# QY-H00/attention-interpolation-diffusion

Hardware: AMD Instinct MI355X
Metric: interpolation-frames/sec (50-step) (higher is better)
Workload: dtype bf16

## Files before the change

attention-interpolation-diffusion_amd/csrc/aid_attn.hip:

```cpp
#include <stdio.h>
#include <stdlib.h>

#include <type_traits>

#include "aid_common.hpp"
#include "aid_kernels.hpp"

namespace aid {

constexpr int KT = 64;
constexpr int VLD = KT + 8;

struct AttnKParams {
    AidAttnArgs a;
    int32_t nqb;
    float   c2;
    int32_t q_iters;
    int32_t skip_single;
};

constexpr int RES_KEYS = 96;
constexpr int RES_VLD = RES_KEYS + 8;
constexpr int RES_SLACK = 64;

// ... 915 lines not shown
                    if (dv < D) {
                        f32x4 v;
#pragma unroll
                        for (int e = 0; e < 4; ++e) v[e] = res[j][d][4 * g + e] * osc;
                        if (a.accumulate) {
                            const f32x4 old = up4<T>(*reinterpret_cast<const T4*>(orow + dv));
                            v += old;
                        }
                        *reinterpret_cast<T4*>(orow + dv) = cvt4<T>(v);
                    }
                }
        }
    }
    if (RES) {
#pragma unroll
        for (int j = 0; j < QB; ++j)
#pragma unroll
            for (int ks = 0; ks < NQK; ++ks) qf[j][ks] = qn[j][ks];
    }
    }
}

template <typename T, int D, int MODE, int NW, int QB, bool PIPE, bool RES = false, bool BIAS = false>
static hipError_t launch_variant(const AttnKParams& p, hipStream_t stream) {
    constexpr int DK = (D + 15) / 16 * 16, DV = (D + 31) / 32 * 32;
    constexpr int NREG = MODE == AID_MODE_PLAIN ? 1 : MODE == AID_MODE_INNER ? 2 : 3;
    const size_t smem = RES ? ((size_t)NREG * (RES_KEYS * (DK + 8) + DV * RES_VLD) + RES_SLACK) * sizeof(T)
                            : (size_t)((attn_prefetch(D, NW) || QB > 1) ? 2 : 1) * (KT * (DK + 8) + DV * VLD) * sizeof(T);
    static PerDevice<int> attr_set;
    const hipError_t e =
        set_max_dynamic_lds(attr_set, 0, reinterpret_cast<const void*>(&aid_attn_kernel<T, D, MODE, NW, QB, PIPE, RES, BIAS>), smem);
    if (e != hipSuccess) return e;
    const int grid = p.nqb * p.a.n_frames * p.a.heads;
    hipLaunchKernelGGL((aid_attn_kernel<T, D, MODE, NW, QB, PIPE, RES, BIAS>), dim3(grid), dim3(NW * 64), smem, stream, p);
    return hipGetLastError();
}

static int attn_qb(const AidAttnArgs& a);

static int attn_nw(const AidAttnArgs& a) {
    const int knob = tune(TUNE_ATTN_NW);
    if (a.d > 80) return 4;
    if (attn_qb(a) >= 2) return 4;
    if (knob >= 0) return knob == 8 ? 8 : 4;
    return (a.d == 64 && a.mode == AID_MODE_OUTER && a.l >= 2048) ? 8 : 4;
}

static int attn_qb(const AidAttnArgs& a) {
    const int force = tune(TUNE_ATTN_QB);
    if (a.d != 40 || a.mode != AID_MODE_PLAIN) return 1;
    if (force == 1 || force == 2) return force;
    return (a.d == 40 && a.mode == AID_MODE_PLAIN && a.s >= 2048 && a.l >= 1024) ? 2 : 1;
}

static bool attn_pipe(const AidAttnArgs& a) {
    const int knob = tune(TUNE_ATTN_PIPE);
    const bool built = a.d == 40 || (a.d == 64 && a.mode == AID_MODE_PLAIN);
    if (!built || a.l < 192) return false;
    return knob > 0;
}

constexpr int RES_CHUNKS_MAX = 8;
static bool attn_res(const AidAttnArgs& a) {
    const int knob = tune(TUNE_ATTN_RES);
    if (a.d > 80 || a.l > RES_KEYS) return false;
    if (knob >= 0) return knob != 0;
    return a.d == 40;
}

template <typename T, int D, int MODE>
static hipError_t launch_order(const AttnStep& st, const AttnKParams& p, hipStream_t stream) {
    constexpr bool SMALL = D <= 80, QB2 = D == 40 && MODE == AID_MODE_PLAIN, CAN_PIPE = D == 40 || (D == 64 && MODE == AID_MODE_PLAIN);
    if (st.bias)             return launch_variant<T, D, MODE, 4, 1, false, false, true>(p, stream);
    if (SMALL && st.res)     return launch_variant<T, D, MODE, 4, 1, false, SMALL>(p, stream);
    if (QB2 && st.qb == 2)   return launch_variant<T, D, MODE, 4, QB2 ? 2 : 1, false>(p, stream);
    if (SMALL && st.nw == 8) return launch_variant<T, D, MODE, SMALL ? 8 : 4, 1, false>(p, stream);
    if (CAN_PIPE && st.pipe) return launch_variant<T, D, MODE, 4, 1, CAN_PIPE>(p, stream);
    const bool base = st.nw == 4 && st.qb == 1 && !st.pipe && !st.res;
    return base ? launch_variant<T, D, MODE, 4, 1, false>(p, stream) : hipErrorInvalidValue;
}

template <typename T>
static hipError_t launch_order(const AttnStep& st, const AttnKParams& p, hipStream_t stream) {
    static_assert(AID_MODE_PLAIN == 0 && AID_MODE_INNER == 1 && AID_MODE_OUTER == 2, "mode index");
    typedef hipError_t (*Fn)(const AttnStep&, const AttnKParams&, hipStream_t);
    static const Fn by_d_mode[4][3] = {{launch_order<T, 40, 0>, launch_order<T, 40, 1>, launch_order<T, 40, 2>},
                                       {launch_order<T, 64, 0>, launch_order<T, 64, 1>, launch_order<T, 64, 2>},
                                       {launch_order<T, 80, 0>, launch_order<T, 80, 1>, launch_order<T, 80, 2>},
                                       {launch_order<T, 160, 0>, launch_order<T, 160, 1>, launch_order<T, 160, 2>}};
    const int di = p.a.d == 40 ? 0 : p.a.d == 64 ? 1 : p.a.d == 80 ? 2 : p.a.d == 160 ? 3 : -1;
    return di < 0 ? hipErrorInvalidValue : by_d_mode[di][p.a.mode](st, p, stream);
}

template <typename T>
__global__ __launch_bounds__(256) void aid_lerp_kv_kernel(const T* __restrict__ k, const T* __restrict__ vt,
                                                          T* __restrict__ k2, T* __restrict__ vt2,
                                                          const float* __restrict__ coef, int n_frames, int begin,
                                                          int end, int64_t k_fs, int64_t vt_fs) {
    typedef typename Vec<T>::v8 T8;
    const int fr = blockIdx.y;
    const float c = coef[fr];
    if (c <= 0.f || c >= 1.f) return;
    const int64_t nk8 = k_fs / 8, nv8 = vt_fs / 8;
    for (int64_t i = (int64_t)blockIdx.x * blockDim.x + threadIdx.x; i < nk8 + nv8; i += (int64_t)gridDim.x * blockDim.x) {
        const bool isk = i < nk8;
        const int64_t j = isk ? i : i - nk8;
        const T* src = isk ? k : vt;
        const int64_t fs = isk ? k_fs : vt_fs;
        const f32x8 x0 = up8<T>(*reinterpret_cast<const T8*>(src + begin * fs + j * 8));
        const f32x8 x1 = up8<T>(*reinterpret_cast<const T8*>(src + end * fs + j * 8));
        f32x8 y;
#pragma unroll
        for (int e = 0; e < 8; ++e) y[e] = fmaf(c, x1[e], (1.f - c) * x0[e]);
        *reinterpret_cast<T8*>((isk ? k2 : vt2) + fr * fs + j * 8) = cvt8<T>(y);
    }
}

hipError_t lerp_kv_launch(const void* k, const void* vt, void* k2, void* vt2, const float* coef, int n_frames, int begin,
                          int end, int64_t k_fs, int64_t vt_fs, int dtype, hipStream_t stream) {
    const int64_t n8 = (k_fs + vt_fs) / 8;
    const int bx = (int)((n8 + 255) / 256 < 1024 ? (n8 + 255) / 256 : 1024);
    dim3 grid(bx > 0 ? bx : 1, n_frames);
    if (dtype == AID_DTYPE_F16)
        hipLaunchKernelGGL(aid_lerp_kv_kernel<f16>, grid, dim3(256), 0, stream, (const f16*)k, (const f16*)vt, (f16*)k2,
                           (f16*)vt2, coef, n_frames, begin, end, k_fs, vt_fs);
    else
        hipLaunchKernelGGL(aid_lerp_kv_kernel<bf16>, grid, dim3(256), 0, stream, (const bf16*)k, (const bf16*)vt,
                           (bf16*)k2, (bf16*)vt2, coef, n_frames, begin, end, k_fs, vt_fs);
    return hipGetLastError();
}

bool attn_head_dim_supported(int d) { return d == 40 || d == 64 || d == 80 || d == 160; }

AttnPlan plan_attn(const AidAttnArgs& a) {
    const char* const mode = a.mode == AID_MODE_PLAIN ? "plain" : a.mode == AID_MODE_INNER ? "inner" : "outer";
    const char* const dt = a.dtype == AID_DTYPE_F16 ? "f16" : "bf16";
    AttnPlan pl;
    AttnStep* st = &pl.step[0];
    pl.n_single = a.mode == AID_MODE_PLAIN ? a.n_frames : a.n_plain + ((a.fused && a.n_frames - a.n_plain >= 2) ? 2 : 0);
    if (a.dtype == AID_DTYPE_F32) {
        st->engine = AttnEngine::F32;
        snprintf(st->label, sizeof(st->label), "aid_attn_f32<d%d,%s>", a.d, mode);
        snprintf(pl.variant, sizeof(pl.variant), "aid_attn_f32");
        return pl;
    }
    const int v2 = tune(TUNE_ATTN_V2);
    if (!a.bias && tune(TUNE_ATTN_TX) != 0 && v2 != 1 && attn_tx_supported(a)) {
        st->engine = AttnEngine::Tx;
        snprintf(st->label, sizeof(st->label), "aid_attn_tx<%s,d64,%s>", dt, mode);
        snprintf(pl.variant, sizeof(pl.variant), "aid_attn_tx<d64,%s>", mode);
        return pl;
    }
    const bool alone = a.mode == AID_MODE_PLAIN || (a.l % 512 == 0 && (a.mode == AID_MODE_OUTER || (a.k2 && a.vt2)));
    const bool dflt = a.l >= ((a.mode == AID_MODE_PLAIN || (a.mode == AID_MODE_OUTER && !a.fused)) ? 2048 : 1024);
    if (!a.bias && attn_pp_supported(a) && (alone || pl.n_single > 0) &&
        (v2 == 1 || (v2 < 0 && alone && dflt))) {
        const char* const kind = a.mode == AID_MODE_PLAIN ? "" : a.mode == AID_MODE_OUTER ? ",outer" : ",inner";
        st->engine = AttnEngine::Pp;
        st->share = alone ? AttnShare::All : AttnShare::Single;
        snprintf(st->label, sizeof(st->label), "aid_attn_pp<%s,d64%s>", dt, alone ? kind : ",riders");
        snprintf(pl.variant, sizeof(pl.variant), "aid_attn_pp<d64%s>", kind);
        if (alone) return pl;
        st = &pl.step[pl.n_steps++];
        st->share = AttnShare::Rest;
    }
    if (a.bias) st->bias = true;
    else if (attn_res(a)) st->res = true;
    else if (attn_qb(a) == 2) st->qb = 2;
    else if (attn_nw(a) == 8) st->nw = 8;
    else if (attn_pipe(a)) st->pipe = true;
    const int rows = 32 * st->nw * st->qb;
    const int nqb = (a.s + rows - 1) / rows;
    st->nqb = nqb;
    if (st->res) {
        int chunks = nqb / 2 < 1 ? 1 : nqb / 2 > RES_CHUNKS_MAX ? RES_CHUNKS_MAX : nqb / 2;
        if (tune(TUNE_ATTN_RES_CHUNKS) > 0) chunks = tune(TUNE_ATTN_RES_CHUNKS);
        st->nqb = nqb < chunks ? nqb : chunks;
        st->q_iters = (nqb + st->nqb - 1) / st->nqb;
    }
    snprintf(st->label, sizeof(st->label), "aid_attn<%s,d%d,%s,%s%s>", dt, a.d, mode, st->res ? "res" : st->nw == 8 ? "nw8" : "nw4",
             st->bias ? ",bias" : st->qb == 2 ? ",qb2" : st->pipe ? ",pipe" : "");
    snprintf(pl.variant, sizeof(pl.variant), "%s", st->label);
    return pl;
}

hipError_t launch_attn_plan(const AidAttnArgs& a, const AttnStep& st, hipStream_t stream) {
    switch (st.engine) {
        case AttnEngine::F32: return attn_f32_launch(a, stream);
        case AttnEngine::Tx:  return attn_tx_launch(a, stream);
        case AttnEngine::Pp:  return attn_pp_launch(a, stream, st.share == AttnShare::All);
        case AttnEngine::Order: break;
    }
    AttnKParams p = {a, st.nqb, a.softmax_scale * 1.4426950408889634f, st.q_iters, st.share == AttnShare::Rest ? 1 : 0};
    if (tune(TUNE_ATTN_ORDER) == 0) p.a.n_plain = 0;
    return a.dtype == AID_DTYPE_F16 ? launch_order<f16>(st, p, stream) : launch_order<bf16>(st, p, stream);
}

}
```

attention-interpolation-diffusion_amd/csrc/aid_attn_pp.hip:

```cpp
#include <type_traits>

#include "aid_common.hpp"
#include "aid_kernels.hpp"

namespace aid {

namespace {

constexpr int PKT = 64;
constexpr int PTILE = 8192;
constexpr int PSTAGE = 2 * PTILE;
constexpr int PNS = 8;

struct AttnPPParams {
    AidAttnArgs a;
    int32_t nqb;
    int32_t multi;
    int32_t persist;
    int32_t hv_lo, hv_hi, hv_units;
    float   c2;
#ifdef AID_ABLATIONS
    int32_t abl;
#endif
};

typedef __amdgpu_buffer_rsrc_t Rsrc;

template <typename T>
__device__ __forceinline__ float dot2_ones(uint32_t w, float acc);
template <>
__device__ __forceinline__ float dot2_ones<bf16>(uint32_t w, float acc) {
    typedef __bf16 b2 __attribute__((ext_vector_type(2)));
    b2 one;
    one[0] = (__bf16)1.0f; one[1] = (__bf16)1.0f;
    return __builtin_amdgcn_fdot2_f32_bf16(__builtin_bit_cast(b2, w), one, acc, false);
}
template <>
__device__ __forceinline__ float dot2_ones<f16>(uint32_t w, float acc) {
    typedef _Float16 h2 __attribute__((ext_vector_type(2)));
    h2 one;
    one[0] = (_Float16)1.0f; one[1] = (_Float16)1.0f;
    return __builtin_amdgcn_fdot2(__builtin_bit_cast(h2, w), one, acc, false);
}

template <int N>
__device__ __forceinline__ void wait_vm() {
    asm volatile("s_waitcnt vmcnt(%0)" ::"n"(N) : "memory");
}
__device__ __forceinline__ void slot_barrier() {
    __builtin_amdgcn_sched_barrier(0);
    __builtin_amdgcn_s_barrier();
    __builtin_amdgcn_sched_barrier(0);
}

template <typename T, int MODE>
__global__ __launch_bounds__(512) void aid_attn_pp_kernel(const AttnPPParams p) {
    typedef typename Vec<T>::v8 T8;
    typedef typename Vec<T>::v4 T4;
    constexpr int D = 64;
    constexpr float XTH = std::is_same<T, f16>::value ? 15.0f : 60.0f;
    constexpr bool SUMM = std::is_same<T, bf16>::value;
    constexpr float XB = SUMM ? XTH - 1.f : 0.f;
    typedef short s16x4 __attribute__((ext_vector_type(4)));
    extern __shared__ __attribute__((aligned(16))) char smem[];

#ifdef AID_ABLATIONS
    long long tl[6];
    tl[0] = clock64();
#endif
    const AidAttnArgs& a = p.a;
    const int tid = threadIdx.x, lane = tid & 63;
    const int wave = __builtin_amdgcn_readfirstlane(tid >> 6);
    const int grp = wave >> 2;
    const int l31 = lane & 31, hi = lane >> 5;

    const int nt = a.l / PKT;
    const int n_items = p.nqb * a.n_frames * a.heads;
    const int n_heavy = a.n_frames - a.n_plain;
    const bool hf = p.multi && a.n_plain > 0 && n_heavy > 0;
    const int xcd = blockIdx.x & 7, wx = blockIdx.x >> 3, WX = gridDim.x >> 3;
    const int nhf = p.hv_hi - p.hv_lo;
    int pb = 0, npx = 0;
    if (p.persist) {
        const int np = a.heads * p.nqb, q = np >> 3, r = np & 7;
        pb = xcd < r ? xcd * (q + 1) : r * (q + 1) + (xcd - r) * q;
        npx = q + (xcd < r ? 1 : 0);
    }
    auto item_lid = [&](int j) __attribute__((always_inline)) {
        if (!p.persist) {
            if (j != 0) return n_items;
            return hf ? heavy_first((int)blockIdx.x, n_items, n_heavy * p.nqb, a.n_frames * p.nqb) : xcd_remap((int)blockIdx.x, n_items);
        }
        const int nhx = npx * nhf, nlx = npx * (a.n_frames - nhf);
        const int hq = nhx / WX, hr = nhx % WX;
        const int hc = hq + (wx < hr ? 1 : 0);
        int t, fr;
        if (j < hc) {
            t = wx + j * WX;
            fr = p.hv_lo + t / npx;
        } else {
            const int jj = j - hc;
            const int ndef = hr > 0 ? WX - hr : 0;
            const int p2 = min(nlx, p.hv_units * ndef);
            const int c1 = (hr > 0 && wx >= hr) ? max(min(p.hv_units * (wx - hr + 1), p2) - p.hv_units * (wx - hr), 0) : 0;
            if (jj < c1) {
                t = p.hv_units * (wx - hr) + jj;
            } else {
                t = p2 + wx + (jj - c1) * WX;
                if (t >= nlx) return n_items;
            }
            const int fi = t / npx;
            fr = fi < p.hv_lo ? fi : fi + nhf;
        }
        const int pi = pb + t % npx;
        return ((pi / p.nqb) * a.n_frames + fr) * p.nqb + pi % p.nqb;
    };
    const int row_b = a.begin, row_e = a.end;
    int N_fr = 0, N_h = 0, N_q0 = 0, N_nseg = 1, N_ks0 = 0, N_ks1 = 0, N_ks2 = 0, N_vs0 = 0, N_vs1 = 0, N_vs2 = 0, N_t2 = 0;
    int N_park = -1, N_swap = -1;
    float N_wb = 0.f, N_we = 1.f;
    bool N_skip = false;
    auto plan = [&](int lid) __attribute__((always_inline)) {
        const int qb = lid % p.nqb;
        N_fr = (lid / p.nqb) % a.n_frames;
        N_h = lid / (p.nqb * a.n_frames);
        N_q0 = (qb * 8 + wave) * 32;
        const int kvf = a.kv_map ? a.kv_map[N_fr] : N_fr;
        int seg0 = kvf, seg1 = 0;
        N_nseg = 1; N_t2 = 0; N_park = -1; N_swap = -1; N_wb = 0.f; N_we = 1.f; N_skip = false;
        if (MODE != AID_MODE_PLAIN) {
            const float cf = a.coef[N_fr];
            const bool single = cf < 0.f || (a.fused && ((cf == 0.f && kvf == row_b) || (cf == 1.f && kvf == row_e)));
            if (!single) {
                N_skip = !p.multi;
                const bool both = cf != 0.f && cf != 1.f;
                const int side = row_b + (cf == 1.f ? 1 : 0) * (row_e - row_b);
                const int fz = a.fused ? 1 : 0;
                if (MODE == AID_MODE_OUTER) {
                    N_nseg = fz + (both ? 2 : 1);
                    const int first = both ? row_b : side;
                    seg0 = fz * kvf + (1 - fz) * first;
                    seg1 = fz * first + (1 - fz) * row_e;
                    if (both) { N_wb = 1.f - cf; N_we = cf; N_park = fz ? 1 : -1; N_swap = fz + 1; }
                } else {
                    N_nseg = fz + 1;
                    const int mix = both ? N_fr : side;
                    seg0 = fz * kvf + (1 - fz) * mix;
                    seg1 = mix;
                    N_t2 = both ? (fz ? 2 : 1) : 0;
                }
            }
        }
        const int kh = N_h * D * 2, vh = N_h * D * a.ldvt * 2;
        N_ks0 = seg0 * (int)a.k_fs * 2 + kh;  N_ks1 = seg1 * (int)a.k_fs * 2 + kh;  N_ks2 = row_e * (int)a.k_fs * 2 + kh;
        N_vs0 = seg0 * (int)a.vt_fs * 2 + vh; N_vs1 = seg1 * (int)a.vt_fs * 2 + vh; N_vs2 = row_e * (int)a.vt_fs * 2 + vh;
    };
    int fr, h, q0, nseg, ks0, ks1, ks2, vs0, vs1, vs2, t2mask, park_at, swap_at, NT;
    float w_b, w_e;
    auto adopt = [&]() __attribute__((always_inline)) {
        fr = N_fr; h = N_h; q0 = N_q0; nseg = N_nseg; ks0 = N_ks0; ks1 = N_ks1; ks2 = N_ks2; vs0 = N_vs0; vs1 = N_vs1; vs2 = N_vs2;
        t2mask = N_t2; park_at = N_park; swap_at = N_swap; w_b = N_wb; w_e = N_we;
        NT = nseg * nt;
    };
    {
        const int first = item_lid(0);
        if (first >= n_items) return;
        plan(first);
    }
    if (N_skip) return;
    adopt();

    T8 qf[4];
    auto scale_q = [&]() __attribute__((always_inline)) {
        if (!a.q_prescaled) {
#pragma unroll
            for (int ks = 0; ks < 4; ++ks) {
                f32x8 t = up8<T>(qf[ks]);
#pragma unroll
                for (int e = 0; e < 8; ++e) t[e] *= p.c2;
                qf[ks] = cvt8<T>(t);
            }
        }
    };
    {
        const int qr = min(q0 + l31, a.s - 1);
        const T* qrow = reinterpret_cast<const T*>(a.q) + (int64_t)fr * a.q_fs + (int64_t)qr * a.ldq + h * D;
#pragma unroll
        for (int ks = 0; ks < 4; ++ks) qf[ks] = *reinterpret_cast<const T8*>(qrow + ks * 16 + hi * 8);
        scale_q();
    }

    const Rsrc rk = __builtin_amdgcn_make_buffer_rsrc(const_cast<void*>(a.k), 0, 0x7fffffff, 0x00020000);
    const Rsrc rv = __builtin_amdgcn_make_buffer_rsrc(const_cast<void*>(a.vt), 0, 0x7fffffff, 0x00020000);
    const Rsrc rk2 = __builtin_amdgcn_make_buffer_rsrc(const_cast<void*>(a.k2), 0, 0x7fffffff, 0x00020000);
    const Rsrc rv2 = __builtin_amdgcn_make_buffer_rsrc(const_cast<void*>(a.vt2), 0, 0x7fffffff, 0x00020000);
    const Rsrc rq = __builtin_amdgcn_make_buffer_rsrc(const_cast<void*>(a.q), 0, 0x7fffffff, 0x00020000);
    char* const qlds = smem + 2 * PNS * PTILE + wave * 4096;
    auto dma_q_next = [&]() __attribute__((always_inline)) {
        const int qr = min(N_q0 + l31, a.s - 1);
        const int vo = qr * (a.ldq * 2) + hi * 16;
        const int so = (int)(((int64_t)N_fr * a.q_fs + N_h * D) * 2);
#pragma unroll
        for (int ks = 0; ks < 4; ++ks)
            __builtin_amdgcn_raw_ptr_buffer_load_lds(rq, (__attribute__((address_space(3))) void*)(qlds + ks * 1024), 16, vo, so + ks * 32, 0, 0);
    };
    const int prow = 8 * wave + (lane >> 3);
    const int pch = (lane & 7) ^ ((prow >> 1) & 7);
    const int kvo = prow * (a.ldk * 2) + pch * 16;
    const int vvo = prow * (a.ldvt * 2) + pch * 16;
    int dk = ks0, dv = vs0, dleft = nt, dseg = 0;
    bool d2 = (t2mask & 1) != 0;
    const int kstep = PKT * a.ldk * 2;
    auto dma_next = [&](int st) __attribute__((always_inline)) {
        char* dst = smem + st * PTILE + wave * 1024;
        if (MODE == AID_MODE_INNER && d2) {
            __builtin_amdgcn_raw_ptr_buffer_load_lds(rk2, (__attribute__((address_space(3))) void*)dst, 16, kvo, dk, 0, 0);
            __builtin_amdgcn_raw_ptr_buffer_load_lds(rv2, (__attribute__((address_space(3))) void*)(dst + PNS * PTILE), 16, vvo, dv, 0, 0);
        } else {
            __builtin_amdgcn_raw_ptr_buffer_load_lds(rk, (__attribute__((address_space(3))) void*)dst, 16, kvo, dk, 0, 0);
            __builtin_amdgcn_raw_ptr_buffer_load_lds(rv, (__attribute__((address_space(3))) void*)(dst + PNS * PTILE), 16, vvo, dv, 0, 0);
        }
        dk += kstep;
        dv += PKT * 2;
        if (__builtin_expect(--dleft == 0, 0)) {
            ++dseg;
            dleft = nt;
            if (dseg < nseg) {
                dk = ks1 + (dseg >= 2 ? ks2 - ks1 : 0);
                dv = vs1 + (dseg >= 2 ? vs2 - vs1 : 0);
                d2 = ((t2mask >> dseg) & 1) != 0;
            } else {
                dk = N_ks0;
                dv = N_vs0;
                d2 = (N_t2 & 1) != 0;
            }
        }
    };
    bool has_next = false;

    const int krow = (l31 & 0x13) | ((l31 & 4) << 1) | ((l31 & 8) >> 1);
    const int kx = hi ^ ((krow >> 1) & 7), vx = hi ^ ((l31 >> 1) & 7);
    const int koff = krow * 128, voff = PNS * PTILE + l31 * 128;
    int kad[4], vad[4];
#pragma unroll
    for (int ks = 0; ks < 4; ++ks) {
        kad[ks] = koff + (((2 * ks) ^ kx) << 4);
        vad[ks] = voff + (((2 * ks) ^ vx) << 4);
    }

    float m = 0.f;
    bool fresh = true;
    f32x16 o[2], sc[2];
    float lsum = 0.f;
    f32x4 lacc = {0.f, 0.f, 0.f, 0.f};
    s16x4 ones4;
#pragma unroll
    for (int i = 0; i < 4; ++i) ones4[i] = 0x3f80;
    asm volatile("" : "+v"(ones4));
    auto get_l = [&]() __attribute__((always_inline)) -> float { return SUMM ? lacc[0] : lsum; };
    auto set_l = [&](float x) __attribute__((always_inline)) {
        if (SUMM) { lacc[0] = x; lacc[1] = x; lacc[2] = x; lacc[3] = x; } else lsum = x;
    };
    T8 pf[4];
    f32x16 cneg;
    f32x16 po[2];
    float pl = 0.f, pm = 0.f;
#pragma unroll
    for (int r = 0; r < 16; ++r) { o[0][r] = 0.f; o[1][r] = 0.f; cneg[r] = 0.f; }
    if (MODE == AID_MODE_OUTER) {
#pragma unroll
        for (int r = 0; r < 16; ++r) { po[0][r] = 0.f; po[1][r] = 0.f; }
    }
    asm volatile("" : "+v"(cneg));
#pragma unroll
    for (int i = 0; i < 4; ++i) pf[i] = zero8<T>();

#ifdef AID_ABLATIONS
    long long tmark = clock64();
    float tacc[4] = {0.f, 0.f, 0.f, 0.f};
    auto stamp = [&](int which) __attribute__((always_inline)) {
        if (p.abl & 16) {
            __builtin_amdgcn_sched_barrier(0);
            const long long now = clock64();
            tacc[which] += (float)(now - tmark);
            tmark = now;
            __builtin_amdgcn_sched_barrier(0);
        }
    };
#define PP_STAMP(i) stamp(i)
#else
#define PP_STAMP(i)
#endif

    auto tie = [&]() __attribute__((always_inline)) {
        asm volatile("" : "+v"(sc[0]), "+v"(sc[1]));
        asm volatile("" : "+v"(o[0]), "+v"(o[1]));
        if (SUMM) asm volatile("" : "+v"(lacc));
    };
    auto settle = [&]() __attribute__((always_inline)) {
        tie();
        asm volatile("s_nop 15\n\ts_nop 3" ::: "memory");
        tie();
    };
    T8 kf[4][2], vf[4][2];
    auto lds_k = [&](int st, int ks, int b) __attribute__((always_inline)) {
        return *reinterpret_cast<const T8*>(smem + kad[ks] + (st * PTILE + b * 4096));
    };
    auto lds_v = [&](int st, int kk, int d) __attribute__((always_inline)) {
        return *reinterpret_cast<const T8*>(smem + vad[kk] + (st * PTILE + d * 4096));
    };
    auto pin = []() __attribute__((always_inline)) { __builtin_amdgcn_sched_barrier(0); };

    auto mslot = [&](int sv, int sk) __attribute__((always_inline)) {
#ifdef AID_ABLATIONS
        if (p.abl & 4) {
            asm volatile("" : "+v"(sc[0]), "+v"(sc[1]));
            return;
        }
#endif
        pin();
#pragma unroll
        for (int i = 0; i < 8; ++i) {
            const int ks = i >> 1, b = i & 1;
#ifdef AID_ABLATIONS
            if (!((p.abl & 64) && b))
#endif
            vf[ks][b] = lds_v(sv, ks, b);
            pin();
            sc[b] = mfma32(kf[ks][b], qf[ks], ks ? sc[b] : cneg);
            pin();
        }
#pragma unroll
        for (int i = 0; i < 8; ++i) {
            const int kk = i >> 1, w = i & 1;
            o[w] = mfma32(vf[kk][w], pf[kk], o[w]);
            pin();
            if constexpr (SUMM) {
                const u32x4 w4 = __builtin_bit_cast(u32x4, pf[kk]);
                u32x2 h2;
                h2[0] = w4[2 * w]; h2[1] = w4[2 * w + 1];
                lacc = __builtin_amdgcn_mfma_f32_4x4x4bf16_1k(ones4, __builtin_bit_cast(s16x4, h2), lacc, 0, 0, 0);
                pin();
            }
#ifdef AID_ABLATIONS
            if (!((p.abl & 64) && w))
#endif
            kf[kk][w] = lds_k(sk, kk, w);
            pin();
        }
    };

    constexpr int LEAD = 6;
    auto vslot = [&](int t, bool first) __attribute__((always_inline)) {
#ifdef AID_ABLATIONS
        if (p.abl & 1) {
            if (!(p.abl & 2)) dma_next((t + LEAD) & (PNS - 1));
            fresh = false;
            wait_vm<6>();
            return;
        }
        if (!(p.abl & 2))
#endif
        dma_next((t + LEAD) & (PNS - 1));
        auto exp_tile = [&]() __attribute__((always_inline)) -> float {
            float t0 = 0.f, t1 = 0.f;
#pragma unroll
            for (int b = 0; b < 2; ++b)
#pragma unroll
                for (int u = 0; u < 2; ++u) {
                    f32x8 pv;
#pragma unroll
                    for (int e = 0; e < 8; ++e) pv[e] = __builtin_amdgcn_exp2f(sc[b][8 * u + e]);
                    pf[2 * b + u] = cvt8<T>(pv);
                    const u32x4 w4 = __builtin_bit_cast(u32x4, pf[2 * b + u]);
                    t0 = dot2_ones<T>(w4[0], t0); t1 = dot2_ones<T>(w4[1], t1);
                    t0 = dot2_ones<T>(w4[2], t0); t1 = dot2_ones<T>(w4[3], t1);
                }
            return t0 + t1;
        };
        auto exp_tile_or = [&]() __attribute__((always_inline)) -> uint32_t {
            uint32_t acc = 0;
#pragma unroll
            for (int b = 0; b < 2; ++b)
#pragma unroll
                for (int u = 0; u < 2; ++u) {
                    f32x8 pv;
#pragma unroll
                    for (int e = 0; e < 8; ++e) pv[e] = __builtin_amdgcn_exp2f(sc[b][8 * u + e]);
                    pf[2 * b + u] = cvt8<T>(pv);
                    const u32x4 w4 = __builtin_bit_cast(u32x4, pf[2 * b + u]);
                    acc = (b == 0 && u == 0) ? (w4[0] | w4[1] | w4[2]) | w4[3] : (acc | w4[0] | w4[1]) | (w4[2] | w4[3]);
                }
            return acc;
        };
        auto row_max = [&]() __attribute__((always_inline)) -> float {
            float xm = fmaxf(sc[0][0], sc[0][1]);
#ifdef AID_ABLATIONS
            if (!(p.abl & 8))
#endif
#pragma unroll
            for (int i = 1; i < 16; ++i) xm = fmaxf(fmaxf(xm, sc[i >> 3][(2 * i) & 15]), sc[i >> 3][(2 * i + 1) & 15]);
            return xm;
        };
        auto raise = [&](float xm) __attribute__((always_inline)) {
            settle();
            const float rowmax = max_halves(xm) + XB;
            const float shift = fresh ? rowmax : fmaxf(rowmax, 0.f);
            const float alpha = __builtin_amdgcn_exp2f(-shift);
            m += shift;
#pragma unroll
            for (int r = 0; r < 16; ++r) cneg[r] = -m;
            asm volatile("" : "+v"(cneg));
#pragma unroll
            for (int r = 0; r < 16; ++r) { o[0][r] *= alpha; o[1][r] *= alpha; }
            if (SUMM) lacc *= alpha; else lsum *= alpha;
#pragma unroll
            for (int b = 0; b < 2; ++b)
#pragma unroll
                for (int r = 0; r < 16; ++r) sc[b][r] -= shift;
            fresh = false;
        };
        const bool fr = first && fresh;
        if constexpr (SUMM) {
            const uint32_t orw = fr ? 0u : exp_tile_or();
            if (__builtin_expect(fr || __any((orw & 0x40004000u) != 0u), 0)) {
                raise(row_max());
                exp_tile_or();
            }
        } else {
            float ts = fr ? 0.f : exp_tile();
            if (__builtin_expect(fr || __any(ts > __builtin_amdgcn_exp2f(XTH)), 0)) {
                raise(row_max());
                ts = exp_tile();
            }
            lsum += ts;
        }
        wait_vm<6>();
    };

    auto park = [&]() __attribute__((always_inline)) {
        settle();
#pragma unroll
        for (int r = 0; r < 16; ++r) { po[0][r] = o[0][r]; po[1][r] = o[1][r]; }
        pl = get_l();
        pm = m;
    };
    auto swap_sides = [&]() __attribute__((always_inline)) {
        settle();
        const float lown = get_l();
        const float lrow = lown + other_half(lown);
        const float wb = w_b / lrow;
#pragma unroll
        for (int d = 0; d < 2; ++d)
#pragma unroll
            for (int r = 0; r < 16; ++r) {
                const float rb = o[d][r] * wb;
                o[d][r] = po[d][r];
                po[d][r] = rb;
            }
        set_l(pl);
        const float back = m - pm;
        m = pm;
#pragma unroll
        for (int r = 0; r < 16; ++r) cneg[r] = -m;
        asm volatile("" : "+v"(cneg));
#pragma unroll
        for (int b = 0; b < 2; ++b)
#pragma unroll
            for (int r = 0; r < 16; ++r) sc[b][r] += back;
        if (park_at < 0) fresh = true;
    };

    auto finish = [&]() __attribute__((always_inline)) {
        settle();
#ifdef AID_ABLATIONS
        if (p.abl & (16 | 32)) {
            if (lane == 0 && q0 < a.s) {
                float* dbg = reinterpret_cast<float*>(reinterpret_cast<T*>(a.out) + (int64_t)fr * a.o_fs + (int64_t)q0 * a.ldo + h * D);
                if (p.abl & 16) for (int i = 0; i < 4; ++i) dbg[i] = tacc[i] / (float)NT;
                else { tl[4] = clock64(); for (int i = 1; i < 5; ++i) dbg[i - 1] = (float)(tl[i] - tl[0]); }
            }
            for (int i = 0; i < 4; ++i) tacc[i] = 0.f;
            tmark = clock64();
            return;
        }
#endif
        const float lown = get_l();
        const float inv = w_e / (lown + other_half(lown));
        if (q0 >= a.s) return;
        const float osc = a.out_scale * (a.frame_scale ? a.frame_scale[fr] : 1.f);
        if (MODE == AID_MODE_OUTER) {
            const int q = q0 + l31;
            if (q < a.s) {
                T* orow = reinterpret_cast<T*>(a.out) + (int64_t)fr * a.o_fs + (int64_t)q * a.ldo + h * D;
#pragma unroll
                for (int d = 0; d < 2; ++d)
#pragma unroll
                    for (int g = 0; g < 4; ++g) {
                        const int dv_ = 32 * d + 8 * g + 4 * hi;
                        f32x4 v;
#pragma unroll
                        for (int e = 0; e < 4; ++e) v[e] = (o[d][4 * g + e] * inv + po[d][4 * g + e]) * osc;
                        if (a.accumulate) v += up4<T>(*reinterpret_cast<const T4*>(orow + dv_));
                        *reinterpret_cast<T4*>(orow + dv_) = cvt4<T>(v);
                    }
            }
        } else {
            char* const st = qlds;
            const int wsw = (l31 >> 1) & 7;
#pragma unroll
            for (int d = 0; d < 2; ++d)
#pragma unroll
                for (int g = 0; g < 4; ++g) {
                    f32x4 v;
#pragma unroll
                    for (int e = 0; e < 4; ++e) v[e] = o[d][4 * g + e] * inv * osc;
                    *reinterpret_cast<T4*>(st + l31 * 128 + (((4 * d + g) ^ wsw) << 4) + 8 * hi) = cvt4<T>(v);
                }
            const Rsrc ro = __builtin_amdgcn_make_buffer_rsrc(a.out, 0, 0x7fffffff, 0x00020000);
            const int so = (int)(((int64_t)fr * a.o_fs + h * D) * 2);
            const int rr = lane >> 3, cc = lane & 7;
#pragma unroll
            for (int i = 0; i < 4; ++i) {
                const int row = rr + 8 * i;
                T8 v = *reinterpret_cast<const T8*>(st + row * 128 + ((cc ^ ((row >> 1) & 7)) << 4));
                const int q = q0 + row;
                const int vo = (min(q, a.s - 1) * a.ldo + cc * 8) * 2;
                if (a.accumulate) v = cvt8<T>(up8<T>(v) + up8<T>(__builtin_bit_cast(T8, __builtin_amdgcn_raw_buffer_load_b128(ro, vo, so, 0))));
                if (q < a.s) __builtin_amdgcn_raw_buffer_store_b128(__builtin_bit_cast(u32x4, v), ro, vo, so, 0);
            }
        }
    };

#pragma unroll
    for (int t = 0; t < LEAD; ++t)
        dma_next(t);
#ifdef AID_ABLATIONS
    if (p.abl & 32) { tl[1] = clock64(); asm volatile("" :: "v"(qf[0]), "v"(qf[3])); }
#endif
    wait_vm<6>();
#ifdef AID_ABLATIONS
    if (p.abl & 32) tl[2] = clock64();
#endif
    slot_barrier();
    if (grp == 1) slot_barrier();
#pragma unroll
    for (int i = 0; i < 8; ++i) kf[i >> 1][i & 1] = lds_k(0, i >> 1, i & 1);
    f32x16 zacc;
#pragma unroll
    for (int r = 0; r < 16; ++r) zacc[r] = 0.f;
#ifdef AID_ABLATIONS
    if (!(p.abl & 4))
#endif
    {
#pragma unroll
        for (int i = 0; i < 8; ++i) sc[i & 1] = mfma32(kf[i >> 1][i & 1], qf[i >> 1], (i >> 1) ? sc[i & 1] : zacc);
        pin();
#pragma unroll
        for (int i = 0; i < 8; ++i) kf[i >> 1][i & 1] = lds_k(1, i >> 1, i & 1);
    }
    settle();
    slot_barrier();
#ifdef AID_ABLATIONS
    if (p.abl & 32) tl[3] = clock64();
#endif
#pragma nounroll
    for (int j = 0;; ++j) {
        const int vbn = item_lid(j + 1);
        has_next = vbn < n_items;
        if (has_next) {
            plan(vbn);
            dma_q_next();
        }
#pragma nounroll
        for (int sgi = 0; sgi < (MODE == AID_MODE_PLAIN ? 1 : nseg); ++sgi) {
            if (MODE == AID_MODE_OUTER) {
                if (sgi == park_at) park();
                if (sgi == swap_at) swap_sides();
            }
            const int t_end = (sgi + 1) * nt;
            for (int t8 = sgi * nt; t8 < t_end; t8 += 8) {
#pragma unroll
                for (int i = 0; i < 8; ++i) {
                    const int t = t8 + i;
                    if (t >= t_end) break;
                    PP_STAMP(3);
                    vslot(t, i == 0);
                    if (i == 7 && __builtin_expect(has_next && t == NT - 1, 0)) {
#pragma unroll
                        for (int ks = 0; ks < 4; ++ks) qf[ks] = *reinterpret_cast<const T8*>(qlds + ks * 1024 + lane * 16);
                        scale_q();
                        m = 0.f;
#pragma unroll
                        for (int r = 0; r < 16; ++r) cneg[r] = 0.f;
                        asm volatile("" : "+v"(cneg));
                    }
                    PP_STAMP(0);
                    slot_barrier();
                    PP_STAMP(1);
                    mslot(i, (i + 2) & 7);
                    tie();
                    PP_STAMP(2);
                    slot_barrier();
                }
            }
        }
        finish();
        if (!has_next) break;
        fresh = true;
        set_l(0.f);
        pl = 0.f;
        pm = 0.f;
#pragma unroll
        for (int r = 0; r < 16; ++r) { o[0][r] = 0.f; o[1][r] = 0.f; }
        if (MODE == AID_MODE_OUTER) {
#pragma unroll
            for (int r = 0; r < 16; ++r) { po[0][r] = 0.f; po[1][r] = 0.f; }
        }
        adopt();
        dseg = 0;
    }
    wait_vm<0>();
    if (grp == 0) slot_barrier();
}

}

bool attn_pp_supported(const AidAttnArgs& a) {
    const int64_t lim = 1ll << 31;
    const int64_t kb = (int64_t)a.n_kv * a.k_fs * 2, vb = (int64_t)a.n_kv * a.vt_fs * 2;
    const int64_t k2b = a.mode == AID_MODE_INNER ? (int64_t)a.n_frames * a.k_fs * 2 : 0;
    const int64_t v2b = a.mode == AID_MODE_INNER ? (int64_t)a.n_frames * a.vt_fs * 2 : 0;
    const int64_t qb = (int64_t)a.n_frames * a.q_fs * 2, ob = (int64_t)a.n_frames * a.o_fs * 2;
    const uintptr_t al = reinterpret_cast<uintptr_t>(a.k) | reinterpret_cast<uintptr_t>(a.vt) | reinterpret_cast<uintptr_t>(a.k2) |
                         reinterpret_cast<uintptr_t>(a.vt2) | reinterpret_cast<uintptr_t>(a.out);
    return a.d == 64 && a.l % PKT == 0 && a.l >= 2 * PKT && a.ldk % 8 == 0 && a.ldvt % 8 == 0 && a.k_fs % 8 == 0 && a.vt_fs % 8 == 0 &&
           (al & 15) == 0 && kb < lim && vb < lim && k2b < lim && v2b < lim && qb < lim && ob < lim && a.ldo % 8 == 0 && a.o_fs % 8 == 0;
}

hipError_t attn_pp_launch(const AidAttnArgs& a, hipStream_t stream, bool multi) {
    AttnPPParams p;
    p.a = a;
    p.multi = multi ? 1 : 0;
    p.nqb = (a.s + 255) / 256;
    p.c2 = a.softmax_scale * 1.4426950408889634f;
#ifdef AID_ABLATIONS
    p.abl = tune(TUNE_ATTN_RES_CHUNKS) > 100 ? tune(TUNE_ATTN_RES_CHUNKS) - 100 : 0;
#endif
    const size_t smem = (size_t)PNS * PSTAGE + 8 * 4096;
    static PerDevice<int> attr_set[2];
    const int ti = a.dtype == AID_DTYPE_F16 ? 0 : 1;
    if (a.mode < AID_MODE_PLAIN || a.mode > AID_MODE_OUTER) return hipErrorInvalidValue;
    const void* fns[2][3] = {
        {reinterpret_cast<const void*>(&aid_attn_pp_kernel<f16, AID_MODE_PLAIN>), reinterpret_cast<const void*>(&aid_attn_pp_kernel<f16, AID_MODE_INNER>),
         reinterpret_cast<const void*>(&aid_attn_pp_kernel<f16, AID_MODE_OUTER>)},
        {reinterpret_cast<const void*>(&aid_attn_pp_kernel<bf16, AID_MODE_PLAIN>), reinterpret_cast<const void*>(&aid_attn_pp_kernel<bf16, AID_MODE_INNER>),
         reinterpret_cast<const void*>(&aid_attn_pp_kernel<bf16, AID_MODE_OUTER>)}};
    static_assert(AID_MODE_PLAIN == 0 && AID_MODE_INNER == 1 && AID_MODE_OUTER == 2, "mode index");
    const void* fn = fns[ti][a.mode];
    const hipError_t e = set_max_dynamic_lds(attr_set[ti], a.mode, fn, smem);
    if (e != hipSuccess) return e;
    const int items = p.nqb * a.n_frames * a.heads;
    static PerDevice<int> cus;
    int* ncu = cus.slot();
    if (!ncu) return hipErrorInvalidDevice;
    if (*ncu == 0) {
        int dev = 0;
        if (hipGetDevice(&dev) != hipSuccess || hipDeviceGetAttribute(ncu, hipDeviceAttributeMultiprocessorCount, dev) != hipSuccess) *ncu = 256;
    }
    const int knob = tune(TUNE_ATTN_PIPE);
    p.persist = ((multi || a.mode == AID_MODE_PLAIN) && (a.l / PKT) % 8 == 0 && items > *ncu && *ncu % 8 == 0 && knob != 0) ? 1 : 0;
    const int n_aid = a.n_frames - a.n_plain;
    p.hv_lo = p.hv_hi = 0;
    p.hv_units = 1;
    if (a.mode == AID_MODE_OUTER && n_aid > 2) { p.hv_lo = 1; p.hv_hi = n_aid - 1; p.hv_units = a.fused ? 3 : 2; }
    if (a.mode == AID_MODE_INNER && a.fused && n_aid > 2) { p.hv_lo = 1; p.hv_hi = n_aid - 1; p.hv_units = 2; }
    const int grid = p.persist ? *ncu : items;
    void* kargs[] = {const_cast<AttnPPParams*>(&p)};
    return hipLaunchKernel(fn, dim3(grid), dim3(512), kargs, smem, stream);
}

}
```

attention-interpolation-diffusion_amd/csrc/aid_kernels.hpp:

```cpp
#pragma once
#include <hip/hip_runtime.h>
#include <stdint.h>
#include "../../include/aid_hip.h"

namespace aid {

struct GemmDesc {
    const void* a;
    const void* b;
    void*       c;
    const void* bias;
    const void* residual;
    int32_t m, n, k;
    int32_t lda, ldb, ldc;
    int32_t batch;
    float   scale;
    int64_t stride_a, stride_b, stride_c;
    const float* ln_stats;
    const float* ln_colsum;
    const float* ln_shift;
    int32_t ln_side;
    int32_t trans_rows;
    int64_t stride_stats;
};

struct GemmGroup {
    GemmDesc p[AID_GEMM_MAX_PROBLEMS];
    int32_t  tile_start[AID_GEMM_MAX_PROBLEMS + 1];
    int32_t  n_problems;
    int32_t  interleave;
};

struct GemmLRDesc {
    const void* a;
    const void* b;
    int32_t k, lda, ldb;
    int32_t side;
    int64_t stride_a, stride_b;
    const float* row_scale;
};
struct GemmLR {
    GemmLRDesc p[AID_GEMM_MAX_PROBLEMS];
};
struct NoLR {};

template <typename V4>
__device__ __forceinline__ void lr_row_scale4(V4& v, const float* __restrict__ gain, int side, int m, int n, int N) {
    const float gm = gain[side == 1 ? m : min(n, N - 1)];
#pragma unroll
    for (int e = 0; e < 4; ++e) {
        float t = v[e] * (side == 1 || e == 0 ? gm : gain[min(n + e, N - 1)]);
        asm volatile("" : "+v"(t));
        v[e] = t;
    }
}
template <int NB, int MB, typename ACC>
__device__ __forceinline__ void lr_row_scale(ACC (&acc)[NB][MB], const float* __restrict__ gain, int side, int m, int n, int M, int N) {
    if (side == 1) {
#pragma unroll
        for (int j = 0; j < MB; ++j) {
            const float gm = gain[min(m + 32 * j, M - 1)];
#pragma unroll
            for (int i = 0; i < NB; ++i)
#pragma unroll
                for (int r = 0; r < 16; ++r) {
                    float t = acc[i][j][r] * gm;
                    asm volatile("" : "+v"(t));
                    acc[i][j][r] = t;
                }
        }
    } else {
#pragma unroll
        for (int i = 0; i < NB; ++i)
#pragma unroll
            for (int gq = 0; gq < 4; ++gq)
#pragma unroll
                for (int e = 0; e < 4; ++e) {
                    const float gn = gain[min(n + 32 * i + 8 * gq + e, N - 1)];
#pragma unroll
                    for (int j = 0; j < MB; ++j) {
                        float t = acc[i][j][4 * gq + e] * gn;
                        asm volatile("" : "+v"(t));
                        acc[i][j][4 * gq + e] = t;
                    }
                }
    }
}

int fill_tile_start(GemmGroup& g, int bm, int bn);

struct GemmSide {
    GemmDesc p[4];
    int32_t  tile_start[5];
    int32_t  n;
    int32_t  tiles;
    int32_t  pad_tiles;
};

enum Tune {
    TUNE_GEMM_VARIANT = 0,
    TUNE_GEMM_PP,
    TUNE_GEMM_TRI,
    TUNE_ATTN_NW,
    TUNE_ATTN_QB,
    TUNE_ATTN_PIPE,
    TUNE_ATTN_RES,
    TUNE_ATTN_RES_CHUNKS,
    TUNE_ATTN_ORDER,
    TUNE_ATTN_V2,
    TUNE_CU_SHARE,
    TUNE_GEMM_RS,
    TUNE_ATTN_TX,
    TUNE_ATTN_TX_TILES,
    TUNE_GEMM_LS,
    TUNE_COUNT
};
int tune(int id);

hipError_t gemm_group_launch(GemmGroup& g, int dtype, hipStream_t stream, const char** variant = nullptr, const char** symbol = nullptr,
                             int cu_share = 0, GemmLR* lr = nullptr);

bool       gemm_rs_supported(const GemmGroup& g, int ncu, bool ignore_size);
hipError_t gemm_rs_launch(const GemmGroup& g, int dtype, int ncu, hipStream_t stream);

hipError_t gemm_f32_launch(GemmGroup& g, hipStream_t stream, const GemmLR* lr = nullptr);
hipError_t attn_f32_launch(const AidAttnArgs& a, hipStream_t stream);
hipError_t lerp_kv_f32_launch(const void* k, const void* vt, void* k2, void* vt2, const float* coef, int n_frames, int begin,
                              int end, int64_t k_fs, int64_t vt_fs, hipStream_t stream);

enum class AttnEngine { F32, Tx, Pp, Order };
enum class AttnShare { All = 0, Single = 1, Rest = 2 };
struct AttnStep {
    AttnEngine engine = AttnEngine::Order;
    AttnShare  share = AttnShare::All;
    int  nw = 4, qb = 1;
    bool pipe = false, res = false, bias = false;
    int  nqb = 0, q_iters = 1;
    char label[64] = "";
};
struct AttnPlan {
    int      n_steps = 1;
    AttnStep step[2];
    int      n_single = 0;
    char     variant[64] = "";
};
AttnPlan   plan_attn(const AidAttnArgs& a);
hipError_t launch_attn_plan(const AidAttnArgs& a, const AttnStep& st, hipStream_t stream);
bool       attn_pp_supported(const AidAttnArgs& a);
hipError_t attn_pp_launch(const AidAttnArgs& a, hipStream_t stream, bool multi);
bool       attn_tx_supported(const AidAttnArgs& a);
hipError_t attn_tx_launch(const AidAttnArgs& a, hipStream_t stream);
bool       attn_head_dim_supported(int d);
hipError_t lerp_kv_launch(const void* k, const void* vt, void* k2, void* vt2, const float* coef, int n_frames, int begin,
                          int end, int64_t k_fs, int64_t vt_fs, int dtype, hipStream_t stream);
hipError_t layernorm_launch(const void* x, const void* gamma, const void* beta, void* y, int64_t rows, int c, float eps,
                            int dtype, hipStream_t stream);
hipError_t ln_stats_launch(const void* x, float* stats, int64_t rows, int c, float eps, int dtype, hipStream_t stream);
hipError_t ln_fold_launch(const void* w, const void* gamma, const void* beta, void* w_folded, float* colsum, float* shift,
                          int rows, int c, int dtype, hipStream_t stream);
hipError_t dora_gain_launch(const void* w, const void* a_pack, const void* b_pack, const void* magnitude, float* gain, int n_out,
                            int n_in, int ldw, int rank, int dtype, hipStream_t stream);
bool       layernorm_width_supported(int c);

}
```

Measured before the change: 4.004.

## Extend persistent pp attention to plain mode at L>=1024 and defer group barriers

The attention planner now picks the persistent pipelined kernel for plain-mode attention at key lengths of 1024 and up whenever persistent scheduling applies, instead of only at 2048 and up. Inside the kernel, per-item scheduling math is hoisted out of the item loop and items are returned as (head, frame, qblock) tuples to avoid divide/modulo work. Small per-frame tables are read through constant-address-space loads so they go through the scalar path. The second wave group defers its final slot barrier across item boundaries to overlap finishing one item with starting the next. It adds a safety check that the output buffer does not alias those tables, plus debug timestamping kept behind the ablation flag.

After: 4.075 (median of 6 runs). +1.8%, better.

```diff
diff --git a/attention-interpolation-diffusion_amd/csrc/aid_attn.hip b/attention-interpolation-diffusion_amd/csrc/aid_attn.hip
--- a/attention-interpolation-diffusion_amd/csrc/aid_attn.hip
+++ b/attention-interpolation-diffusion_amd/csrc/aid_attn.hip
@@ -1091,7 +1091,8 @@
         return pl;
     }
     const bool alone = a.mode == AID_MODE_PLAIN || (a.l % 512 == 0 && (a.mode == AID_MODE_OUTER || (a.k2 && a.vt2)));
-    const bool dflt = a.l >= ((a.mode == AID_MODE_PLAIN || (a.mode == AID_MODE_OUTER && !a.fused)) ? 2048 : 1024);
+    const bool dflt = a.l >= ((a.mode == AID_MODE_PLAIN || (a.mode == AID_MODE_OUTER && !a.fused)) ? 2048 : 1024) ||
+                      (a.mode == AID_MODE_PLAIN && a.l >= 1024 && attn_pp_persistent(a, true, nullptr));
     if (!a.bias && attn_pp_supported(a) && (alone || pl.n_single > 0) &&
         (v2 == 1 || (v2 < 0 && alone && dflt))) {
         const char* const kind = a.mode == AID_MODE_PLAIN ? "" : a.mode == AID_MODE_OUTER ? ",outer" : ",inner";
diff --git a/attention-interpolation-diffusion_amd/csrc/aid_attn_pp.hip b/attention-interpolation-diffusion_amd/csrc/aid_attn_pp.hip
--- a/attention-interpolation-diffusion_amd/csrc/aid_attn_pp.hip
+++ b/attention-interpolation-diffusion_amd/csrc/aid_attn_pp.hip
@@ -42,6 +42,17 @@
     one[0] = (_Float16)1.0f; one[1] = (_Float16)1.0f;
     return __builtin_amdgcn_fdot2(__builtin_bit_cast(h2, w), one, acc, false);
 }
+
+template <typename V>
+__device__ __forceinline__ V ld_uniform(const V* ptr, int i) {
+    return reinterpret_cast<const __attribute__((address_space(4))) V*>(reinterpret_cast<uintptr_t>(ptr))[i];
+}
+
+#ifdef AID_ABLATIONS
+#define PP_LDU(ptr, i) ((p.abl & 512) ? (ptr)[i] : ld_uniform(ptr, i))
+#else
+#define PP_LDU(ptr, i) ld_uniform(ptr, i)
+#endif
 
 template <int N>
 __device__ __forceinline__ void wait_vm() {
@@ -86,50 +97,58 @@
         pb = xcd < r ? xcd * (q + 1) : r * (q + 1) + (xcd - r) * q;
         npx = q + (xcd < r ? 1 : 0);
     }
-    auto item_lid = [&](int j) __attribute__((always_inline)) {
+    int hc = 0, hr = 0, c1 = 0, p2 = 0, nlx = 0;
+    if (p.persist) {
+        const int nhx = npx * nhf;
+        nlx = npx * (a.n_frames - nhf);
+        const int hq = nhx / WX;
+        hr = nhx % WX;
+        hc = hq + (wx < hr ? 1 : 0);
+        const int ndef = hr > 0 ? WX - hr : 0;
+        p2 = min(nlx, p.hv_units * ndef);
+        c1 = (hr > 0 && wx >= hr) ? max(min(p.hv_units * (wx - hr + 1), p2) - p.hv_units * (wx - hr), 0) : 0;
+    }
+    struct Item { int h, fr, qb; bool ok; };
+    auto item_at = [&](int j) __attribute__((always_inline)) -> Item {
+        const Item none = {0, 0, 0, false};
         if (!p.persist) {
-            if (j != 0) return n_items;
-            return hf ? heavy_first((int)blockIdx.x, n_items, n_heavy * p.nqb, a.n_frames * p.nqb) : xcd_remap((int)blockIdx.x, n_items);
-        }
-        const int nhx = npx * nhf, nlx = npx * (a.n_frames - nhf);
-        const int hq = nhx / WX, hr = nhx % WX;
-        const int hc = hq + (wx < hr ? 1 : 0);
+            if (j != 0) return none;
+            const int lid = hf ? heavy_first((int)blockIdx.x, n_items, n_heavy * p.nqb, a.n_frames * p.nqb) : xcd_remap((int)blockIdx.x, n_items);
+            if (lid >= n_items) return none;
+            return Item{lid / (p.nqb * a.n_frames), (lid / p.nqb) % a.n_frames, lid % p.nqb, true};
+        }
         int t, fr;
         if (j < hc) {
             t = wx + j * WX;
             fr = p.hv_lo + t / npx;
         } else {
             const int jj = j - hc;
-            const int ndef = hr > 0 ? WX - hr : 0;
-            const int p2 = min(nlx, p.hv_units * ndef);
-            const int c1 = (hr > 0 && wx >= hr) ? max(min(p.hv_units * (wx - hr + 1), p2) - p.hv_units * (wx - hr), 0) : 0;
             if (jj < c1) {
                 t = p.hv_units * (wx - hr) + jj;
             } else {
                 t = p2 + wx + (jj - c1) * WX;
-                if (t >= nlx) return n_items;
+                if (t >= nlx) return none;
             }
             const int fi = t / npx;
             fr = fi < p.hv_lo ? fi : fi + nhf;
         }
         const int pi = pb + t % npx;
-        return ((pi / p.nqb) * a.n_frames + fr) * p.nqb + pi % p.nqb;
+        return Item{pi / p.nqb, fr, pi % p.nqb, true};
     };
     const int row_b = a.begin, row_e = a.end;
     int N_fr = 0, N_h = 0, N_q0 = 0, N_nseg = 1, N_ks0 = 0, N_ks1 = 0, N_ks2 = 0, N_vs0 = 0, N_vs1 = 0, N_vs2 = 0, N_t2 = 0;
     int N_park = -1, N_swap = -1;
     float N_wb = 0.f, N_we = 1.f;
     bool N_skip = false;
-    auto plan = [&](int lid) __attribute__((always_inline)) {
-        const int qb = lid % p.nqb;
-        N_fr = (lid / p.nqb) % a.n_frames;
-        N_h = lid / (p.nqb * a.n_frames);
-        N_q0 = (qb * 8 + wave) * 32;
-        const int kvf = a.kv_map ? a.kv_map[N_fr] : N_fr;
+    auto plan = [&](const Item it) __attribute__((always_inline)) {
+        N_fr = it.fr;
+        N_h = it.h;
+        N_q0 = (it.qb * 8 + wave) * 32;
+        const int kvf = a.kv_map ? PP_LDU(a.kv_map, N_fr) : N_fr;
         int seg0 = kvf, seg1 = 0;
         N_nseg = 1; N_t2 = 0; N_park = -1; N_swap = -1; N_wb = 0.f; N_we = 1.f; N_skip = false;
         if (MODE != AID_MODE_PLAIN) {
-            const float cf = a.coef[N_fr];
+            const float cf = PP_LDU(a.coef, N_fr);
             const bool single = cf < 0.f || (a.fused && ((cf == 0.f && kvf == row_b) || (cf == 1.f && kvf == row_e)));
             if (!single) {
                 N_skip = !p.multi;
@@ -163,8 +182,8 @@
         NT = nseg * nt;
     };
     {
-        const int first = item_lid(0);
-        if (first >= n_items) return;
+        const Item first = item_at(0);
+        if (!first.ok) return;
         plan(first);
     }
     if (N_skip) return;
@@ -288,8 +307,24 @@
         }
     };
 #define PP_STAMP(i) stamp(i)
+    long long bt0 = 0;
+    uint32_t bt[11];
+    for (int i = 0; i < 11; ++i) bt[i] = 0;
+    int64_t boff = -1;
+    bool barm = false;
+    auto bstamp = [&](int which) __attribute__((always_inline)) {
+        if (barm) {
+            __builtin_amdgcn_sched_barrier(0);
+            const long long now = clock64();
+            if (which == 0) bt0 = now;
+            bt[which] = (uint32_t)(now - bt0);
+            __builtin_amdgcn_sched_barrier(0);
+        }
+    };
+#define PP_BSTAMP(i) bstamp(i)
 #else
 #define PP_STAMP(i)
+#define PP_BSTAMP(i) do {} while (0)
 #endif
 
     auto tie = [&]() __attribute__((always_inline)) {
@@ -488,7 +523,7 @@
         const float lown = get_l();
         const float inv = w_e / (lown + other_half(lown));
         if (q0 >= a.s) return;
-        const float osc = a.out_scale * (a.frame_scale ? a.frame_scale[fr] : 1.f);
+        const float osc = a.out_scale * (a.frame_scale ? PP_LDU(a.frame_scale, fr) : 1.f);
         if (MODE == AID_MODE_OUTER) {
             const int q = q0 + l31;
             if (q < a.s) {
@@ -564,14 +599,17 @@
 #ifdef AID_ABLATIONS
     if (p.abl & 32) tl[3] = clock64();
 #endif
+    const bool defer = p.persist && grp == 1;
 #pragma nounroll
     for (int j = 0;; ++j) {
-        const int vbn = item_lid(j + 1);
-        has_next = vbn < n_items;
+        const Item nxt = item_at(j + 1);
+        has_next = nxt.ok;
         if (has_next) {
-            plan(vbn);
+            plan(nxt);
             dma_q_next();
         }
+        if (defer && j > 0) slot_barrier();
+        PP_BSTAMP(2);
 #pragma nounroll
         for (int sgi = 0; sgi < (MODE == AID_MODE_PLAIN ? 1 : nseg); ++sgi) {
             if (MODE == AID_MODE_OUTER) {
@@ -596,17 +634,33 @@
                         asm volatile("" : "+v"(cneg));
                     }
                     PP_STAMP(0);
+                    if (i < 4) PP_BSTAMP(3 + 2 * i);
                     slot_barrier();
                     PP_STAMP(1);
+                    if (i < 4) PP_BSTAMP(4 + 2 * i);
+#ifdef AID_ABLATIONS
+                    if (i == 3 && barm) {
+                        barm = false;
+                        if (q0 < a.s) boff = (int64_t)fr * a.o_fs + (int64_t)q0 * a.ldo + h * D;
+                    }
+#endif
                     mslot(i, (i + 2) & 7);
                     tie();
                     PP_STAMP(2);
-                    slot_barrier();
+                    if (!(i == 7 && defer && t == NT - 1)) slot_barrier();
                 }
             }
         }
+#ifdef AID_ABLATIONS
+        barm = (p.abl & 256) && j == 1 && has_next;
+#endif
+        PP_BSTAMP(0);
         finish();
-        if (!has_next) break;
+        PP_BSTAMP(1);
+        if (!has_next) {
+            if (defer) slot_barrier();
+            break;
+        }
         fresh = true;
         set_l(0.f);
         pl = 0.f;
@@ -621,6 +675,13 @@
         dseg = 0;
     }
     wait_vm<0>();
+#ifdef AID_ABLATIONS
+    if ((p.abl & 256) && boff >= 0 && lane == 0) {
+        uint32_t* dbg = reinterpret_cast<uint32_t*>(reinterpret_cast<T*>(a.out) + boff);
+        dbg[0] = 0x50504254u; dbg[1] = 0x4c494e45u;
+        for (int i = 0; i < 11; ++i) dbg[2 + i] = bt[i];
+    }
+#endif
     if (grp == 0) slot_barrier();
 }
 
@@ -634,8 +695,28 @@
     const int64_t qb = (int64_t)a.n_frames * a.q_fs * 2, ob = (int64_t)a.n_frames * a.o_fs * 2;
     const uintptr_t al = reinterpret_cast<uintptr_t>(a.k) | reinterpret_cast<uintptr_t>(a.vt) | reinterpret_cast<uintptr_t>(a.k2) |
                          reinterpret_cast<uintptr_t>(a.vt2) | reinterpret_cast<uintptr_t>(a.out);
+    const uintptr_t o0 = reinterpret_cast<uintptr_t>(a.out), o1 = o0 + (uintptr_t)ob;
+    for (const void* rec : {(const void*)a.coef, (const void*)a.frame_scale, (const void*)a.kv_map}) {
+        const uintptr_t r0 = reinterpret_cast<uintptr_t>(rec);
+        if (rec && r0 < o1 && o0 < r0 + 4 * (uintptr_t)a.n_frames) return false;
+    }
     return a.d == 64 && a.l % PKT == 0 && a.l >= 2 * PKT && a.ldk % 8 == 0 && a.ldvt % 8 == 0 && a.k_fs % 8 == 0 && a.vt_fs % 8 == 0 &&
            (al & 15) == 0 && kb < lim && vb < lim && k2b < lim && v2b < lim && qb < lim && ob < lim && a.ldo % 8 == 0 && a.o_fs % 8 == 0;
+}
+
+bool attn_pp_persistent(const AidAttnArgs& a, bool multi, int* n_cu) {
+    static PerDevice<int> cus;
+    int* ncu = cus.slot();
+    if (n_cu) *n_cu = ncu ? 0 : -1;
+    if (!ncu) return false;
+    if (*ncu == 0) {
+        int dev = 0;
+        if (hipGetDevice(&dev) != hipSuccess || hipDeviceGetAttribute(ncu, hipDeviceAttributeMultiprocessorCount, dev) != hipSuccess) *ncu = 256;
+    }
+    if (n_cu) *n_cu = *ncu;
+    const int items = ((a.s + 255) / 256) * a.n_frames * a.heads;
+    const int knob = tune(TUNE_ATTN_PIPE);
+    return (multi || a.mode == AID_MODE_PLAIN) && (a.l / PKT) % 8 == 0 && items > *ncu && *ncu % 8 == 0 && knob != 0;
 }
 
 hipError_t attn_pp_launch(const AidAttnArgs& a, hipStream_t stream, bool multi) {
@@ -660,22 +741,15 @@
     const void* fn = fns[ti][a.mode];
     const hipError_t e = set_max_dynamic_lds(attr_set[ti], a.mode, fn, smem);
     if (e != hipSuccess) return e;
-    const int items = p.nqb * a.n_frames * a.heads;
-    static PerDevice<int> cus;
-    int* ncu = cus.slot();
-    if (!ncu) return hipErrorInvalidDevice;
-    if (*ncu == 0) {
-        int dev = 0;
-        if (hipGetDevice(&dev) != hipSuccess || hipDeviceGetAttribute(ncu, hipDeviceAttributeMultiprocessorCount, dev) != hipSuccess) *ncu = 256;
-    }
-    const int knob = tune(TUNE_ATTN_PIPE);
-    p.persist = ((multi || a.mode == AID_MODE_PLAIN) && (a.l / PKT) % 8 == 0 && items > *ncu && *ncu % 8 == 0 && knob != 0) ? 1 : 0;
+    int ncu = 0;
+    p.persist = attn_pp_persistent(a, multi, &ncu) ? 1 : 0;
+    if (ncu <= 0) return hipErrorInvalidDevice;
     const int n_aid = a.n_frames - a.n_plain;
     p.hv_lo = p.hv_hi = 0;
     p.hv_units = 1;
     if (a.mode == AID_MODE_OUTER && n_aid > 2) { p.hv_lo = 1; p.hv_hi = n_aid - 1; p.hv_units = a.fused ? 3 : 2; }
     if (a.mode == AID_MODE_INNER && a.fused && n_aid > 2) { p.hv_lo = 1; p.hv_hi = n_aid - 1; p.hv_units = 2; }
-    const int grid = p.persist ? *ncu : items;
+    const int grid = p.persist ? ncu : p.nqb * a.n_frames * a.heads;
     void* kargs[] = {const_cast<AttnPPParams*>(&p)};
     return hipLaunchKernel(fn, dim3(grid), dim3(512), kargs, smem, stream);
 }
diff --git a/attention-interpolation-diffusion_amd/csrc/aid_kernels.hpp b/attention-interpolation-diffusion_amd/csrc/aid_kernels.hpp
--- a/attention-interpolation-diffusion_amd/csrc/aid_kernels.hpp
+++ b/attention-interpolation-diffusion_amd/csrc/aid_kernels.hpp
@@ -148,6 +148,7 @@
 hipError_t launch_attn_plan(const AidAttnArgs& a, const AttnStep& st, hipStream_t stream);
 bool       attn_pp_supported(const AidAttnArgs& a);
 hipError_t attn_pp_launch(const AidAttnArgs& a, hipStream_t stream, bool multi);
+bool       attn_pp_persistent(const AidAttnArgs& a, bool multi, int* n_cu);
 bool       attn_tx_supported(const AidAttnArgs& a);
 hipError_t attn_tx_launch(const AidAttnArgs& a, hipStream_t stream);
 bool       attn_head_dim_supported(int d);
```
